# jfdev001/algebraic-multigrid

Hardware: AMD Instinct MI355X
Metric: V-cycles/sec, 2D Poisson N=4096^2 (fine-grid smoother HBM GB/s under roofline) (higher is better)
Workload: dtype f64; 1 GPU; 2D 5-point Poisson 4096x4096 (Grid::laplacian/rhs), true Jacobi smoother omega=0.6 2+2 sweeps, 16-level V-cycle, coarsest 511 dofs, fp64, 1xMI355X; smoother has no counterpart in the reference: pinned to the oracle twin; n=4096, dim=2, levels=16, smoother=jacobi, sweeps=2, graph=True, coarse_solve=band-chain (LDS-resident scalar recurrence, half-bandwidth <= 3, bit-exact), layout=dict

## Files before the change

algebraic-multigrid_amd/csrc/kernels.hip:

```cpp
#include <hip/hip_runtime.h>
#include <cstdlib>
#include <stdint.h>

#include <cstdio>
#include <type_traits>
#include <utility>
#include <vector>
#include <algorithm>
#include <cmath>

#include "kernels.hpp"

namespace amg_hip {

__device__ __forceinline__ void lds_barrier() {
  asm volatile("s_waitcnt lgkmcnt(0)\n\ts_barrier" ::: "memory");
}

constexpr bool mode_cheb(int m) { return (m & ~3) == 16; }
constexpr bool mode_jac(int m) { return m == CSR_JACOBI || mode_cheb(m); }
constexpr bool cheb_first(int m) { return (m & 1) != 0; }
constexpr bool cheb_last(int m) { return (m & 2) != 0; }
template <int MODE>
__device__ __forceinline__ double cheb_update(double t, double xi, double di, double alpha, double beta,
// ... 250 lines not shown
      else { if (v > w[2]) w[2] = v; }
    }
  }
#pragma unroll
  for (int a = 0; a < 3; ++a) red[a][threadIdx.x] = w[a];
  __syncthreads();
  for (int h = 128; h > 0; h >>= 1) {
    if ((int)threadIdx.x < h) {
#pragma unroll
      for (int a = 0; a < 3; ++a) red[a][threadIdx.x] = fmax(red[a][threadIdx.x], red[a][threadIdx.x + h]);
    }
    __syncthreads();
  }
  if (threadIdx.x < 3) atomicMax(out + threadIdx.x, (unsigned long long)__double_as_longlong(red[threadIdx.x][0]));
}
__global__ void axis_strength_init_kernel(unsigned long long* out) {
  if (threadIdx.x < 3) out[threadIdx.x] = 0ull;
}
hipError_t launch_axis_strength(int64_t n, int dim, const int64_t dims[3], const int32_t* rowptr, const int32_t* col,
                                const double* val, uint64_t* out, hipStream_t st) {
  if ((dim != 2 && dim != 3) || !dims || dims[0] < 1 || dims[1] < 1 || dims[2] < 1 ||
      n != dims[0] * dims[1] * dims[2] || n >= ((int64_t)1 << 31))
    return hipErrorInvalidValue;
  hipLaunchKernelGGL(axis_strength_init_kernel, dim3(1), dim3(64), 0, st, reinterpret_cast<unsigned long long*>(out));
  hipError_t e = hipGetLastError();
  if (e != hipSuccess) return e;
  hipLaunchKernelGGL(axis_strength_kernel, dim3((unsigned)((n + 255) / 256)), dim3(256), 0, st, (uint32_t)n,
                     (uint32_t)dims[0], (uint32_t)dims[1], rowptr, col, val, reinterpret_cast<unsigned long long*>(out));
  return hipGetLastError();
}

template <int MODE, bool IDX16, bool NT>
__global__ __launch_bounds__(256) void sell_kernel(
    int n, const int64_t* __restrict__ soff, const void* __restrict__ scol_v,
    const double* __restrict__ sval, const double* x, const double* __restrict__ f,
    double* out, double omega, const int32_t* __restrict__ rowid, int row0,
    const double* __restrict__ uH, int nH, int dshift, double* dvec, double alpha) {
  auto corrected = [&](int c) -> double {
    const double xc = x[c];
    const int j = c >> 1;
    const double a = uH[(j >= 1 && j - 1 < nH) ? j - 1 : 0];
    const double b = uH[j < nH ? j : 0];
    double t = 0.0;
    if (c & 1) {
      if (j < nH) t += 1.0 * b;
    } else {
      if (j >= 1 && j - 1 < nH) t += 0.5 * a;
      if (j < nH) t += 0.5 * b;
    }
    return xc + t;
  };
  const int32_t* __restrict__ scol = static_cast<const int32_t*>(scol_v);
  const int16_t* __restrict__ scol16 = static_cast<const int16_t*>(scol_v);
  const int p = row0 + blockIdx.x * 256 + threadIdx.x;
  const int s = p >> 6;
  if ((s << 6) >= n) return;
  const int64_t o0 = soff[s], o1 = soff[s + 1];
  const int w = (int)((o1 - o0) >> 6);
  const int64_t base = o0 + (p & 63);
  int row = p;
  bool live = p < n;
  if (MODE == CSR_GS) {
    row = live ? rowid[p] : -1;
    live = row >= 0;
  }
  const int drow = row + dshift;
  double fi = 0.0, xi = 0.0, di = 0.0;
  if (live) {
    if (MODE != CSR_SPMV) fi = NT ? __builtin_nontemporal_load(f + row) : f[row];
    if (mode_jac(MODE) || MODE == CSR_GS) xi = x[drow];
    if (MODE == CSR_JACOBI_P) xi = corrected(row);
    if (mode_cheb(MODE) && !cheb_first(MODE)) di = NT ? __builtin_nontemporal_load(dvec + row) : dvec[row];
  }
  double acc = (MODE == CSR_RESID) ? fi : 0.0;
  double diag = 0.0;
  auto pass = [&](int j0, auto UU) {
    constexpr int UN = decltype(UU)::value;
    int32_t c[UN];
    double v[UN], xx[UN];
#pragma unroll
    for (int u = 0; u < UN; ++u) {
      const int j = j0 + u < w ? j0 + u : j0;
      const int64_t at = base + ((int64_t)j << 6);
      if (IDX16) {
        const int d = NT ? __builtin_nontemporal_load(scol16 + at) : scol16[at];
        c[u] = (d == -32768) ? -1 : drow + d;
      } else {
        c[u] = NT ? __builtin_nontemporal_load(scol + at) : scol[at];
      }
      v[u] = NT ? __builtin_nontemporal_load(sval + at) : sval[at];
    }
#pragma unroll
    for (int u = 0; u < UN; ++u) {
      if (MODE == CSR_JACOBI_P) xx[u] = corrected(c[u] >= 0 ? c[u] : 0);
      else xx[u] = x[c[u] >= 0 ? c[u] : 0];
    }
#pragma unroll
    for (int u = 0; u < UN; ++u) {
      if (j0 + u < w && c[u] >= 0) {
        if (MODE == CSR_RESID) {
          acc -= v[u] * xx[u];
        } else if (mode_jac(MODE) || MODE == CSR_GS || MODE == CSR_JACOBI_P) {
          if (c[u] == drow) diag = v[u];
          else acc += v[u] * xx[u];
        } else {
          acc += v[u] * xx[u];
        }
      }
    }
  };
  if (w == 0) {
  } else if (w <= 3) pass(0, std::integral_constant<int, 3>{});
  else if (w <= 5) pass(0, std::integral_constant<int, 5>{});
  else if (w <= 7) pass(0, std::integral_constant<int, 7>{});
  else if (w <= 9) pass(0, std::integral_constant<int, 9>{});
  else
    for (int j0 = 0; j0 < w; j0 += 8) pass(j0, std::integral_constant<int, 8>{});
  if (live) {
    double res;
    bool store = true;
    if (MODE == CSR_RESID || MODE == CSR_SPMV) {
      res = acc;
    } else if (MODE == CSR_JACOBI || MODE == CSR_JACOBI_P) {
      res = (diag == 0.0) ? xi : xi + omega * ((fi - acc) / diag - xi);
    } else if (mode_cheb(MODE)) {
      double dn;
      res = cheb_update<MODE>((diag == 0.0) ? xi : (fi - acc) / diag, xi, di, alpha, omega, dn);
      if (!cheb_last(MODE)) {
        if (NT) __builtin_nontemporal_store(dn, dvec + row);
        else dvec[row] = dn;
      }
    } else if (MODE == CSR_GS) {
      res = (fi - acc) / diag;
      store = diag != 0.0;
    } else {
      const double d = fi - acc;
      res = d * d;
    }
    if (store) {
      if (NT && MODE != CSR_GS) __builtin_nontemporal_store(res, out + row);
      else out[row] = res;
    }
  }
}

template <int MODE>
static hipError_t launch_sell_mode(int64_t n, int idx16, const int64_t* soff,
                                   const void* scol, const double* sval, const double* x,
                                   const double* f, double* out, double omega,
                                   const int32_t* rowid, int64_t row0, int64_t count,
                                   const double* uH, int64_t nH, hipStream_t st,
                                   int64_t diag_shift = 0, double* dvec = nullptr, double alpha = 0.0) {
  const unsigned grid = (unsigned)((count + 255) / 256);
#define AMG_SELL_LAUNCH(I16, NTF)                                                              \
  hipLaunchKernelGGL((sell_kernel<MODE, I16, NTF>), dim3(grid), dim3(256), 0, st, (int)n, soff, \
                     scol, sval, x, f, out, omega, rowid, (int)row0, uH, (int)nH, (int)diag_shift, dvec, alpha)
  switch (idx16 & 3) {
    case 0: AMG_SELL_LAUNCH(false, false); break;
    case 1: AMG_SELL_LAUNCH(true, false); break;
    case 2: AMG_SELL_LAUNCH(false, true); break;
    default: AMG_SELL_LAUNCH(true, true); break;
  }
#undef AMG_SELL_LAUNCH
  return hipGetLastError();
}
hipError_t launch_sell(int mode, int64_t n, int idx16, const int64_t* soff,
                       const void* scol, const double* sval, const double* x,
                       const double* f, double* out, double omega, int64_t diag_shift,
                       hipStream_t st) {
  if (n <= 0) return hipSuccess;
  if (n >= ((int64_t)1 << 31) - 256 || diag_shift >= ((int64_t)1 << 30)) return hipErrorInvalidValue;
  switch (mode) {
    case CSR_RESID: return launch_sell_mode<CSR_RESID>(n, idx16, soff, scol, sval, x, f, out, omega, nullptr, 0, n, nullptr, 0, st, diag_shift);
    case CSR_JACOBI: return launch_sell_mode<CSR_JACOBI>(n, idx16, soff, scol, sval, x, f, out, omega, nullptr, 0, n, nullptr, 0, st, diag_shift);
    case CSR_SPMV: return launch_sell_mode<CSR_SPMV>(n, idx16, soff, scol, sval, x, f, out, omega, nullptr, 0, n, nullptr, 0, st, diag_shift);
    case CSR_RSSQ: return launch_sell_mode<CSR_RSSQ>(n, idx16, soff, scol, sval, x, f, out, omega, nullptr, 0, n, nullptr, 0, st, diag_shift);
  }
  return hipErrorInvalidValue;
}

hipError_t launch_sell_cheb(int64_t n, int idx16, const int64_t* soff, const void* scol, const double* sval,
                            const double* x, const double* f, double* out, const ChebStep& c, hipStream_t st) {
  if (n <= 0) return hipSuccess;
  if (n >= ((int64_t)1 << 31) - 256 || !c.d || x == out) return hipErrorInvalidValue;
#define AMG_SELL_CHEB(FI, LA)                                                                                \
  return launch_sell_mode<cheb_kernel_mode(FI, LA)>(n, idx16, soff, scol, sval, x, f, out, c.beta, nullptr, 0, n, \
                                                    nullptr, 0, st, 0, c.d, c.alpha)
  if (c.first && c.last) AMG_SELL_CHEB(true, true);
  if (c.first) AMG_SELL_CHEB(true, false);
  if (c.last) AMG_SELL_CHEB(false, true);
  AMG_SELL_CHEB(false, false);
#undef AMG_SELL_CHEB
}

hipError_t launch_sell_jacobi_prolong(int64_t n, int idx16, const int64_t* soff,
                                      const void* scol, const double* sval, const double* u,
                                      const double* uH, int64_t nH, const double* f, double* out,
                                      double omega, hipStream_t st) {
  if (n <= 0) return hipSuccess;
  if (n >= ((int64_t)1 << 31) - 256 || nH < 1) return hipErrorInvalidValue;
  return launch_sell_mode<CSR_JACOBI_P>(n, idx16, soff, scol, sval, u, f, out, omega, nullptr,
                                        0, n, uH, nH, st);
}

hipError_t launch_sell_gs_color(int64_t n_storage, int ,
                                const int64_t* soff, const int32_t* scol, const double* sval,
                                const int32_t* rowid,
                                int64_t row0, int64_t count, const double* f, double* u,
                                hipStream_t st) {
  if (count <= 0) return hipSuccess;
  if (n_storage >= ((int64_t)1 << 31) - 256 || (row0 & 63)) return hipErrorInvalidValue;
  const int64_t end = row0 + count < n_storage ? row0 + count : n_storage;
  return launch_sell_mode<CSR_GS>(end, 0, soff, scol, sval, u, f, u, 1.0, rowid, row0,
                                  count, nullptr, 0, st);
}

static int g_dict_rows_per_lane = 2;
static int g_xcd_map = 1;
template <int WORDS, int R>
struct DictStream {
  uint64_t cw[R][2];
  uint32_t ty;
  double fi[R], xi[R];
  double di[R];
  bool live[R];
};
template <int MODE, int WORDS, bool NT, int R>
__device__ __forceinline__ void dict_fetch(DictStream<WORDS, R>& s, int row0, int n,
                                           const uint64_t* __restrict__ codes,
                                           const uint8_t* __restrict__ rtype,
                                           const double* __restrict__ f, const double* x,
                                           int dshift, const double* __restrict__ dvec = nullptr) {
  typedef uint64_t u64x2 __attribute__((ext_vector_type(2)));
  typedef double f64x2 __attribute__((ext_vector_type(2)));
  constexpr bool read_d = mode_cheb(MODE) && !cheb_first(MODE);
#pragma unroll
  for (int r = 0; r < R; ++r) {
    s.live[r] = row0 + r < n;
    s.cw[r][0] = s.cw[r][1] = ~(uint64_t)0;
    s.fi[r] = s.xi[r] = s.di[r] = 0.0;
  }
  s.ty = 0xFFFFu;
  if (R == 2 && s.live[R - 1]) {
    if (rtype) {
      s.ty = *reinterpret_cast<const uint16_t*>(rtype + row0);
    } else {
      const u64x2* vp = reinterpret_cast<const u64x2*>(codes + (int64_t)row0 * WORDS);
      const u64x2 a = NT ? __builtin_nontemporal_load(vp) : *vp;
      if (WORDS == 2) {
        const u64x2 b2 = NT ? __builtin_nontemporal_load(vp + 1) : vp[1];
        s.cw[0][0] = a.x; s.cw[0][1] = a.y; s.cw[R - 1][0] = b2.x; s.cw[R - 1][1] = b2.y;
      } else {
        s.cw[0][0] = a.x; s.cw[R - 1][0] = a.y;
      }
    }
    if (MODE != CSR_SPMV) {
      const f64x2* fp = reinterpret_cast<const f64x2*>(f + row0);
      const f64x2 t = NT ? __builtin_nontemporal_load(fp) : *fp;
      s.fi[0] = t.x; s.fi[R - 1] = t.y;
    }
    if (mode_jac(MODE)) { s.xi[0] = x[row0 + dshift]; s.xi[R - 1] = x[row0 + 1 + dshift]; }
    if (read_d) {
      const f64x2* dp = reinterpret_cast<const f64x2*>(dvec + row0);
      const f64x2 t = NT ? __builtin_nontemporal_load(dp) : *dp;
      s.di[0] = t.x; s.di[R - 1] = t.y;
    }
  } else if (s.live[0]) {
    if (rtype) {
      s.ty = 0xFF00u | rtype[row0];
    } else {
      const uint64_t* cp = codes + (int64_t)row0 * WORDS;
      if (WORDS == 2) {
        const u64x2* vp = reinterpret_cast<const u64x2*>(cp);
        const u64x2 t = NT ? __builtin_nontemporal_load(vp) : *vp;
        s.cw[0][0] = t.x; s.cw[0][1] = t.y;
      } else {
        s.cw[0][0] = NT ? __builtin_nontemporal_load(cp) : cp[0];
      }
    }
    if (MODE != CSR_SPMV) s.fi[0] = NT ? __builtin_nontemporal_load(f + row0) : f[row0];
    if (mode_jac(MODE)) s.xi[0] = x[row0 + dshift];
    if (read_d) s.di[0] = NT ? __builtin_nontemporal_load(dvec + row0) : dvec[row0];
  }
}
template <int WORDS>
__device__ __forceinline__ void dict_stage_words(uint64_t* wtab, const uint64_t* __restrict__ rwords) {
#pragma unroll
  for (int k = 0; k < WORDS; ++k) wtab[threadIdx.x * WORDS + k] = rwords[threadIdx.x * WORDS + k];
}
template <int WORDS, int R>
__device__ __forceinline__ void dict_expand(DictStream<WORDS, R>& s, const uint64_t* wtab) {
#pragma unroll
  for (int r = 0; r < R; ++r)
#pragma unroll
    for (int k = 0; k < WORDS; ++k) s.cw[r][k] = wtab[((s.ty >> (8 * r)) & 0xFFu) * WORDS + k];
}
struct DictEntry {
  double a;
  double d;
  int32_t off8;
  int32_t pad[3];
};
template <int MODE>
__device__ __forceinline__ void dict_stage_table(DictEntry* tab, const int32_t* __restrict__ doff,
                                                 const double* __restrict__ dval, int ntab) {
  const int t = threadIdx.x;
  const double v = t < ntab ? dval[t] : 0.0;
  const int32_t o = t < ntab ? doff[t] : 0;
  DictEntry e;
  constexpr bool split = mode_jac(MODE) || MODE == CSR_GS;
  e.a = (split && o == 0) ? 0.0 : v;
  e.d = (split && o == 0 && t < ntab) ? v : 0.0;
  e.off8 = o * 8;
  e.pad[0] = e.pad[1] = e.pad[2] = 0;
  tab[t] = e;
}
template <int MODE, int WORDS, int UN, int R>
__device__ __forceinline__ void dict_rows(const DictStream<WORDS, R>& s, int row0,
                                          const DictEntry* tab, const double* x, double omega,
                                          int dshift, double (&res)[R]) {
  uint32_t c8[R][UN];
  double v[R][UN], vd[R][UN], xx[R][UN];
  bool ok[R][UN];
  const char* xb = reinterpret_cast<const char*>(x);
#pragma unroll
  for (int r = 0; r < R; ++r) {
    const uint32_t drow8 = s.live[r] ? (uint32_t)(row0 + r + dshift) * 8u : 0u;
    const uint32_t w32[4] = {(uint32_t)s.cw[r][0], (uint32_t)(s.cw[r][0] >> 32),
                             (uint32_t)s.cw[r][1], (uint32_t)(s.cw[r][1] >> 32)};
#pragma unroll
    for (int u = 0; u < UN; ++u) {
      const uint32_t code = (w32[u >> 2] >> (8 * (u & 3))) & 0xFFu;
      ok[r][u] = code != 0xFFu;
      c8[r][u] = drow8 + (uint32_t)tab[code].off8;
      v[r][u] = tab[code].a;
      vd[r][u] = (mode_jac(MODE) || MODE == CSR_GS) ? tab[code].d : 0.0;
    }
  }
#pragma unroll
  for (int r = 0; r < R; ++r)
#pragma unroll
    for (int u = 0; u < UN; ++u)
      xx[r][u] = *reinterpret_cast<const double*>(xb + c8[r][u]);
#pragma unroll
  for (int r = 0; r < R; ++r) {
    double acc = (MODE == CSR_RESID) ? s.fi[r] : 0.0;
    double diag = 0.0;
#pragma unroll
    for (int u = 0; u < UN; ++u) {
      double t = v[r][u] * xx[r][u];
      if (mode_jac(MODE) || MODE == CSR_GS) {
        acc += t;
        diag += vd[r][u];
      } else {
        asm volatile("" : "+v"(t));
        t = ok[r][u] ? t : 0.0;
        if (MODE == CSR_RESID) acc -= t;
        else acc += t;
      }
    }
    if (MODE == CSR_RESID || MODE == CSR_SPMV) {
      res[r] = acc;
    } else if (mode_jac(MODE) || MODE == CSR_GS) {
      const bool nod = diag == 0.0;
      double q = (s.fi[r] - acc) / (nod ? 1.0 : diag);
      asm volatile("" : "+v"(q));
      if (MODE == CSR_GS || mode_cheb(MODE)) res[r] = nod ? s.xi[r] : q;
      else res[r] = nod ? s.xi[r] : s.xi[r] + omega * (q - s.xi[r]);
    } else {
      const double d = s.fi[r] - acc;
      res[r] = d * d;
    }
  }
}
template <int UN>
__device__ __forceinline__ bool dict_stencil_can(uint32_t ty, const bool (&live)[2],
                                                 const int32_t* __restrict__ uti) {
  constexpr int PAT = UN == 7 ? 7 : 15;
  const uint32_t t0 = (uint32_t)__builtin_amdgcn_readfirstlane((int)(ty & 0xFFu));
  const bool ok = ty == (t0 | (t0 << 8)) && live[0] && live[1];
  if (t0 == 255u || __builtin_amdgcn_ballot_w64(!ok) != 0) return false;
  return uti[t0 * 18u + 17u] == PAT;
}
template <int MODE, int UN>
__device__ __forceinline__ void dict_rows_stencil(uint32_t ty, const double (&fi)[2],
                                                  const double (&xi)[2], int row0,
                                                  const double* __restrict__ utd,
                                                  const int32_t* __restrict__ uti, const double* x,
                                                  double omega, double (&res)[2]) {
  static_assert(mode_jac(MODE) || MODE == CSR_RESID, "fast path of the hot modes");
  static_assert(UN == 7 || UN == 16, "7-point rows / 15-point rows");
  typedef double f64x2 __attribute__((ext_vector_type(2)));
  constexpr int PAT = UN == 7 ? 7 : 15;
  const uint32_t t0 = (uint32_t)__builtin_amdgcn_readfirstlane((int)(ty & 0xFFu));
  const int32_t* ti = uti + t0 * 18u;
  const double* td = utd + t0 * 33u + (MODE == CSR_RESID ? 16u : 0u);
  const double* xr = x + row0;
  double xx[2][PAT];
  if (PAT == 7) {
    const int g[4] = {0, 1, 5, 6};
#pragma unroll
    for (int k = 0; k < 4; ++k) {
      const f64x2 v = *reinterpret_cast<const f64x2*>(xr + ti[g[k]]);
      xx[0][g[k]] = v.x;
      xx[1][g[k]] = v.y;
    }
    const f64x2 c = *reinterpret_cast<const f64x2*>(xr);
    const double lo = xr[-1], hi = xr[2];
    xx[0][2] = lo;  xx[0][3] = c.x; xx[0][4] = c.y;
    xx[1][2] = c.x; xx[1][3] = c.y; xx[1][4] = hi;
  } else {
#pragma unroll
    for (int k = 0; k < 5; ++k) {
      const double* xc = xr + ti[3 * k + 1];
      const f64x2 c = *reinterpret_cast<const f64x2*>(xc);
      const double lo = xc[-1], hi = xc[2];
      xx[0][3 * k] = lo;  xx[0][3 * k + 1] = c.x; xx[0][3 * k + 2] = c.y;
      xx[1][3 * k] = c.x; xx[1][3 * k + 1] = c.y; xx[1][3 * k + 2] = hi;
    }
  }
#pragma unroll
  for (int r = 0; r < 2; ++r) {
    double acc = (MODE == CSR_RESID) ? fi[r] : 0.0;
#pragma unroll
    for (int u = 0; u < PAT; ++u) {
      const double t = td[u] * xx[r][u];
      if (mode_jac(MODE)) acc += t;
      else acc -= t;
    }
    if (MODE == CSR_RESID) {
      res[r] = acc;
    } else {
      const double diag = td[32];
      const bool nod = diag == 0.0;
      const double q = (fi[r] - acc) / (nod ? 1.0 : diag);
      if (mode_cheb(MODE)) res[r] = nod ? xi[r] : q;
      else res[r] = nod ? xi[r] : xi[r] + omega * (q - xi[r]);
    }
  }
}
template <int WORDS, bool NT, int R>
__device__ __forceinline__ void dict_store(const DictStream<WORDS, R>& s, int row0,
                                           const double (&res)[R], double* out) {
  typedef double f64x2 __attribute__((ext_vector_type(2)));
  if (R == 2 && s.live[R - 1]) {
    f64x2 t;
    t.x = res[0]; t.y = res[R - 1];
    f64x2* op = reinterpret_cast<f64x2*>(out + row0);
    if (NT) __builtin_nontemporal_store(t, op);
    else *op = t;
  } else if (s.live[0]) {
    if (NT) __builtin_nontemporal_store(res[0], out + row0);
    else out[row0] = res[0];
  }
}

__device__ __forceinline__ int xcd_tile(unsigned b, unsigned nb, int on) {
  if (!on) return (int)b;
  if (on >= 16) {
    const unsigned tp = (unsigned)on, s = tp >> 3;
    if (b >= nb / tp * tp) return (int)b;
    const unsigned k = b & 7u, i = b >> 3, p = i / s;
    return (int)(p * tp + k * s + (i - p * s));
  }
  const unsigned k = b & 7u, i = b >> 3, q = nb >> 3, r = nb & 7u;
  return (int)(k * q + (k < r ? k : r) + i);
}
template <int MODE, int WORDS, int UN, bool NT, int R>
__global__ __launch_bounds__(256) void dict_kernel(
    int n, const uint64_t* __restrict__ codes, const uint8_t* __restrict__ rtype,
    const uint64_t* __restrict__ rwords, const int32_t* __restrict__ doff,
    const double* __restrict__ dval, int ntab, const double* x, const double* __restrict__ f,
    double* out, double omega, int dshift, int xcd_map, const double* __restrict__ utd,
    const int32_t* __restrict__ uti, double* dvec, double alpha) {
  __shared__ DictEntry tab[256];
  __shared__ uint64_t wtab[256 * WORDS];
  const int row0 = (xcd_tile(blockIdx.x, gridDim.x, xcd_map) * 256 + (int)threadIdx.x) * R;
  DictStream<WORDS, R> s;
  dict_fetch<MODE, WORDS, NT, R>(s, row0, n, codes, rtype, f, x, dshift, dvec);
  dict_stage_table<MODE>(tab, doff, dval, ntab);
  if (rtype) dict_stage_words<WORDS>(wtab, rwords);
  __syncthreads();
  double res[R];
  bool fast = false;
  if constexpr ((mode_jac(MODE) || MODE == CSR_RESID) && R == 2 && (UN == 7 || UN == 16)) {
    if (utd) fast = dict_stencil_can<UN>(s.ty, s.live, uti);
    if (fast) dict_rows_stencil<MODE, UN>(s.ty, s.fi, s.xi, row0, utd, uti, x, omega, res);
  }
  if (!fast) {
    if (rtype) dict_expand<WORDS, R>(s, wtab);
    dict_rows<MODE, WORDS, UN, R>(s, row0, tab, x, omega, dshift, res);
  }
  if constexpr (mode_cheb(MODE)) {
    double dn[R];
#pragma unroll
    for (int r = 0; r < R; ++r) res[r] = cheb_update<MODE>(res[r], s.xi[r], s.di[r], alpha, omega, dn[r]);
    if (!cheb_last(MODE)) dict_store<WORDS, NT, R>(s, row0, dn, dvec);
  }
  dict_store<WORDS, NT, R>(s, row0, res, out);
}

template <int R>
__device__ __forceinline__ void dict_restrict_tail(int tile, int n, const double* rs, int nH,
                                                   double* __restrict__ fH,
                                                   const double* __restrict__ diagH,
                                                   double* __restrict__ uH1,
                                                   double* __restrict__ uH0, double omega) {
  for (int q = threadIdx.x; q < 128 * R - 1; q += 256) {
    const int j = tile * (128 * R - 1) + q;
    if (j >= nH) break;
    const int64_t i = 2 * (int64_t)j;
    double sum = 0.0;
    if (i < n) sum += 0.5 * rs[2 * q];
    if (i + 1 < n) sum += 1.0 * rs[2 * q + 1];
    if (i + 2 < n) sum += 0.5 * rs[2 * q + 2];
    fH[j] = sum;
    if (uH1) {
      const double xi = 0.0, acc = 0.0;
      const double d = diagH[j];
      uH1[j] = (d == 0.0) ? xi : xi + omega * ((sum - acc) / d - xi);
    } else {
      uH0[j] = 0.0;
    }
  }
}
template <int R>
__device__ __forceinline__ void dict_prolong_tail(int tile, int n, const double* rs, int n_h,
                                                  const double* uh_in, double* uh_out) {
  typedef double f64x2 __attribute__((ext_vector_type(2)));
  const int stride = 256 * R - 2;
#pragma unroll
  for (int r = 0; r < R; ++r) {
    const int q = (int)threadIdx.x * R + r;
    const int j = tile * stride + q;
    if ((q == 0 && tile != 0) || q > stride || j > n) continue;
    double t0 = 0.0, t1 = 0.0;
    const double b = (j < n) ? rs[q] : 0.0;
    if (j >= 1 && j - 1 < n) t0 += 0.5 * rs[q - 1];
    if (j < n) {
      t0 += 0.5 * b;
      t1 += 1.0 * b;
    }
    const int64_t i = 2 * (int64_t)j;
    if (i + 1 < n_h) {
      f64x2 u = *reinterpret_cast<const f64x2*>(uh_in + i);
      u.x = u.x + t0;
      u.y = u.y + t1;
      *reinterpret_cast<f64x2*>(uh_out + i) = u;
    } else if (i < n_h) {
      uh_out[i] = uh_in[i] + t0;
    }
  }
}
template <int WORDS, int UN, bool NT, int R>
__global__ __launch_bounds__(256) void dict_resid_restrict_kernel(
    int n, const uint64_t* __restrict__ codes, const uint8_t* __restrict__ rtype,
    const uint64_t* __restrict__ rwords, const int32_t* __restrict__ doff,
    const double* __restrict__ dval, int ntab, const double* x, const double* __restrict__ f,
    double* r_out, int nH, double* __restrict__ fH, const double* __restrict__ diagH,
    double* __restrict__ uH1, double* __restrict__ uH0, double omega, int xcd_map,
    const double* __restrict__ utd, const int32_t* __restrict__ uti) {
  __shared__ DictEntry tab[256];
  __shared__ uint64_t wtab[256 * WORDS];
  __shared__ double rs[256 * R];
  const int tile = xcd_tile(blockIdx.x, gridDim.x, xcd_map);
  const int row0 = tile * (256 * R - 2) + (int)threadIdx.x * R;
  DictStream<WORDS, R> s;
  dict_fetch<CSR_RESID, WORDS, NT, R>(s, row0, n, codes, rtype, f, x, 0);
  dict_stage_table<CSR_RESID>(tab, doff, dval, ntab);
  if (rtype) dict_stage_words<WORDS>(wtab, rwords);
  __syncthreads();
  double res[R];
  bool fast = false;
  if constexpr (R == 2 && (UN == 7 || UN == 16)) {
    if (utd) fast = dict_stencil_can<UN>(s.ty, s.live, uti);
    if (fast) dict_rows_stencil<CSR_RESID, UN>(s.ty, s.fi, s.xi, row0, utd, uti, x, omega, res);
  }
  if (!fast) {
    if (rtype) dict_expand<WORDS, R>(s, wtab);
    dict_rows<CSR_RESID, WORDS, UN, R>(s, row0, tab, x, omega, 0, res);
  }
  if (r_out) dict_store<WORDS, NT, R>(s, row0, res, r_out);
#pragma unroll
  for (int r = 0; r < R; ++r) rs[threadIdx.x * R + r] = s.live[r] ? res[r] : 0.0;
  __syncthreads();
  dict_restrict_tail<R>(tile, n, rs, nH, fH, diagH, uH1, uH0, omega);
}
template <int WORDS, int UN, bool NT, int R>
__global__ __launch_bounds__(256) void dict_jacobi_prolong_kernel(
    int n, const uint64_t* __restrict__ codes, const uint8_t* __restrict__ rtype,
    const uint64_t* __restrict__ rwords, const int32_t* __restrict__ doff,
    const double* __restrict__ dval, int ntab, const double* x, const double* __restrict__ f,
    double* out, double omega, int n_h, const double* uh_in, double* uh_out, int xcd_map,
    const double* __restrict__ utd, const int32_t* __restrict__ uti) {
  __shared__ DictEntry tab[256];
  __shared__ uint64_t wtab[256 * WORDS];
  __shared__ double rs[256 * R];
  const int tile = xcd_tile(blockIdx.x, gridDim.x, xcd_map);
  const int stride = 256 * R - 2;
  const int row0 = tile * stride + (int)threadIdx.x * R;
  DictStream<WORDS, R> s;
  dict_fetch<CSR_JACOBI, WORDS, NT, R>(s, row0, n, codes, rtype, f, x, 0);
  dict_stage_table<CSR_JACOBI>(tab, doff, dval, ntab);
  if (rtype) dict_stage_words<WORDS>(wtab, rwords);
  __syncthreads();
  double res[R];
  bool fast = false;
  if constexpr (R == 2 && (UN == 7 || UN == 16)) {
    if (utd) fast = dict_stencil_can<UN>(s.ty, s.live, uti);
    if (fast) dict_rows_stencil<CSR_JACOBI, UN>(s.ty, s.fi, s.xi, row0, utd, uti, x, omega, res);
  }
  if (!fast) {
    if (rtype) dict_expand<WORDS, R>(s, wtab);
    dict_rows<CSR_JACOBI, WORDS, UN, R>(s, row0, tab, x, omega, 0, res);
  }
  dict_store<WORDS, NT, R>(s, row0, res, out);
#pragma unroll
  for (int r = 0; r < R; ++r) rs[threadIdx.x * R + r] = s.live[r] ? res[r] : 0.0;
  __syncthreads();
  dict_prolong_tail<R>(tile, n, rs, n_h, uh_in, uh_out);
}

constexpr int PAIR_HB = 66;
constexpr int PAIR_W = 512 + 2 * PAIR_HB;

template <int WORDS, int UN>
__device__ __forceinline__ void dict_pair_stage1(int n, int w0, int hbw, const uint64_t* codes,
                                                 const uint8_t* rtype, const DictEntry* tabJ,
                                                 const uint64_t* wtab, const double* a,
                                                 const double* f, double omega, double* uw,
                                                 double* u_out) {
  const int W = 512 + 2 * hbw;
  for (int base = 0; base < W; base += 512) {
    const int lw = base + (int)threadIdx.x * 2;
    const int row0 = w0 + lw;
    DictStream<WORDS, 2> s;
    const bool inside = row0 >= 0 && lw < W;
    dict_fetch<CSR_JACOBI, WORDS, false, 2>(s, inside ? row0 : 0, inside ? n : 0, codes, rtype, f, a, 0);
    if (rtype) dict_expand<WORDS, 2>(s, wtab);
    double res[2];
    dict_rows<CSR_JACOBI, WORDS, UN, 2>(s, row0, tabJ, a, omega, 0, res);
    if (lw < W) {
      uw[lw] = s.live[0] ? res[0] : 0.0;
      uw[lw + 1] = s.live[1] ? res[1] : 0.0;
    }
    if (u_out && lw >= hbw && lw < hbw + 512) dict_store<WORDS, false, 2>(s, row0, res, u_out);
  }
}
template <int WORDS, int UN>
__global__ __launch_bounds__(256) void dict_pair_down_kernel(
    int n, const uint64_t* __restrict__ codes, const uint8_t* __restrict__ rtype,
    const uint64_t* __restrict__ rwords, const int32_t* __restrict__ doff,
    const double* __restrict__ dval, int ntab, const double* a, const double* __restrict__ f,
    double* u_out, double* r_out, int nH, double* __restrict__ fH,
    const double* __restrict__ diagH, double* __restrict__ uH1, double omega, int hbw,
    int xcd_map) {
  __shared__ DictEntry tabJ[256];
  __shared__ DictEntry tabR[256];
  __shared__ uint64_t wtab[256 * WORDS];
  __shared__ double uw[PAIR_W];
  __shared__ double rs[512];
  const int tile = xcd_tile(blockIdx.x, gridDim.x, xcd_map);
  const int t0 = tile * 510, w0 = t0 - hbw;
  dict_stage_table<CSR_JACOBI>(tabJ, doff, dval, ntab);
  dict_stage_table<CSR_RESID>(tabR, doff, dval, ntab);
  if (rtype) dict_stage_words<WORDS>(wtab, rwords);
  __syncthreads();
  dict_pair_stage1<WORDS, UN>(n, w0, hbw, codes, rtype, tabJ, wtab, a, f, omega, uw, u_out);
  __syncthreads();
  const int row0 = t0 + (int)threadIdx.x * 2;
  DictStream<WORDS, 2> s;
  dict_fetch<CSR_RESID, WORDS, false, 2>(s, row0, n, codes, rtype, f, a, 0);
  if (rtype) dict_expand<WORDS, 2>(s, wtab);
  double res[2];
  dict_rows<CSR_RESID, WORDS, UN, 2>(s, row0 - w0, tabR, uw, omega, 0, res);
  if (r_out) dict_store<WORDS, false, 2>(s, row0, res, r_out);
  rs[threadIdx.x * 2] = s.live[0] ? res[0] : 0.0;
  rs[threadIdx.x * 2 + 1] = s.live[1] ? res[1] : 0.0;
  __syncthreads();
  dict_restrict_tail<2>(tile, n, rs, nH, fH, diagH, uH1, nullptr, omega);
}
template <int WORDS, int UN>
__global__ __launch_bounds__(256) void dict_pair_up_kernel(
    int n, const uint64_t* __restrict__ codes, const uint8_t* __restrict__ rtype,
    const uint64_t* __restrict__ rwords, const int32_t* __restrict__ doff,
    const double* __restrict__ dval, int ntab, const double* a, const double* __restrict__ f,
    double* u_out, double omega, int hbw, int n_h, const double* uh_in, double* uh_out,
    int xcd_map) {
  __shared__ DictEntry tabJ[256];
  __shared__ uint64_t wtab[256 * WORDS];
  __shared__ double uw[PAIR_W];
  __shared__ double rs[512];
  const int tile = xcd_tile(blockIdx.x, gridDim.x, xcd_map);
  const int t0 = tile * 510, w0 = t0 - hbw;
  dict_stage_table<CSR_JACOBI>(tabJ, doff, dval, ntab);
  if (rtype) dict_stage_words<WORDS>(wtab, rwords);
  __syncthreads();
  dict_pair_stage1<WORDS, UN>(n, w0, hbw, codes, rtype, tabJ, wtab, a, f, omega, uw, nullptr);
  __syncthreads();
  const int row0 = t0 + (int)threadIdx.x * 2;
  DictStream<WORDS, 2> s;
  dict_fetch<CSR_RESID, WORDS, false, 2>(s, row0, n, codes, rtype, f, a, 0);
  s.xi[0] = uw[row0 - w0];
  s.xi[1] = uw[row0 - w0 + 1];
  if (rtype) dict_expand<WORDS, 2>(s, wtab);
  double res[2];
  dict_rows<CSR_JACOBI, WORDS, UN, 2>(s, row0 - w0, tabJ, uw, omega, 0, res);
  dict_store<WORDS, false, 2>(s, row0, res, u_out);
  rs[threadIdx.x * 2] = s.live[0] ? res[0] : 0.0;
  rs[threadIdx.x * 2 + 1] = s.live[1] ? res[1] : 0.0;
  __syncthreads();
  dict_prolong_tail<2>(tile, n, rs, n_h, uh_in, uh_out);
}

constexpr int PATCH_TW = 64;
constexpr int PATCH_TH = 42;
constexpr int PATCH_EH = PATCH_TH + 6;
constexpr int PATCH_EC = PATCH_TW + 8;
constexpr int PATCH_NT = 432;
constexpr int PATCH_K = PATCH_EH * PATCH_EC / PATCH_NT;
constexpr int PATCH_BUF = (PATCH_EH + 2) * PATCH_EC;
constexpr int PATCH_MAXTAB = 192;
static_assert(PATCH_EH * PATCH_EC == PATCH_K * PATCH_NT && PATCH_NT % PATCH_EC == 0, "patch geometry");

struct PatchJ { double a, d; };
struct PatchR { double a; int32_t loff, ok; };

struct PatchCells {
  int cell0, row0, lj0, li;
  double f[PATCH_K];
  uint32_t ty[PATCH_K];
  bool live[PATCH_K];
  bool uniform;
  uint32_t tu;
};

struct PatchU {
  double wj[9], wr[9], diag;
#ifdef AMG_PATCH_FASTDIV
  double rdiag;
#endif
  uint32_t rmask, corners;
};
__device__ __forceinline__ void patch_load_u(PatchU& U, uint32_t tu, const double* __restrict__ utabd,
                                             const int32_t* __restrict__ utabi) {
  const double* d = utabd + (size_t)tu * 19;
  const int32_t* i = utabi + (size_t)tu * 2;
#pragma unroll
  for (int e = 0; e < 9; ++e) {
    U.wj[e] = d[e];
    U.wr[e] = d[9 + e];
  }
  U.diag = d[18];
#ifdef AMG_PATCH_FASTDIV
  U.rdiag = 1.0 / (U.diag == 0.0 ? 1.0 : U.diag);
#endif
  U.rmask = (uint32_t)i[0];
  U.corners = (uint32_t)i[1];
}
template <bool RESID, bool CORNERS, bool GS = false, int MASK = -1>
__device__ __forceinline__ void patch_eval_u(const double* buf, int cell0, const PatchU& U,
                                             const double (&f)[PATCH_K], double omega,
                                             double (&res)[PATCH_K]) {
  const double* p = buf + cell0 - PATCH_EC;
  if (!CORNERS && !RESID && U.diag == 0.0) {
#pragma unroll
    for (int k = 0; k < PATCH_K; ++k) res[k] = p[(k + 1) * PATCH_EC];
    return;
  }
  double w[3][3];
#pragma unroll
  for (int r = 0; r < 2; ++r)
#pragma unroll
    for (int c = 0; c < 3; ++c) w[r][c] = (CORNERS || c == 1 || r == 1) ? p[r * PATCH_EC + c - 1] : 0.0;
#pragma unroll
  for (int k = 0; k < PATCH_K; ++k) {
#pragma unroll
    for (int c = 0; c < 3; ++c)
      w[2][c] = (CORNERS || c == 1) ? p[(k + 2) * PATCH_EC + c - 1] : 0.0;
    if (!CORNERS) {
      w[2][0] = p[(k + 2) * PATCH_EC - 1];
      w[2][2] = p[(k + 2) * PATCH_EC + 1];
    }
    const double xi = w[1][1];
    if (RESID) {
      double acc = f[k];
#pragma unroll
      for (int s9 = 0; s9 < 9; ++s9) {
        const int r = s9 / 3, c = s9 % 3;
        if (!CORNERS && r != 1 && c != 1) continue;
        if (MASK >= 0) {
          if ((MASK >> s9) & 1) acc -= U.wr[s9] * w[r][c];
        } else {
          double t = U.wr[s9] * w[r][c];
          t = ((U.rmask >> s9) & 1u) ? t : 0.0;
          acc -= t;
        }
      }
      res[k] = acc;
    } else {
      double acc = 0.0;
#pragma unroll
      for (int s9 = 0; s9 < 9; ++s9) {
        const int r = s9 / 3, c = s9 % 3;
        if (s9 == 4 || (!CORNERS && r != 1 && c != 1)) continue;
        if (MASK >= 0 && !((MASK >> s9) & 1)) continue;
        acc += U.wj[s9] * w[r][c];
      }
      if (CORNERS && U.diag == 0.0) {
        res[k] = xi;
      } else {
#ifdef AMG_PATCH_FASTDIV
        const double nm = f[k] - acc;
        const double q0 = nm * U.rdiag;
        const double r0 = __builtin_fma(-U.diag, q0, nm);
        const double q1 = __builtin_fma(r0, U.rdiag, q0);
        const double r1 = __builtin_fma(-U.diag, q1, nm);
        const double q = __builtin_fma(r1, U.rdiag, q1);
#else
        const double q = (f[k] - acc) / U.diag;
#endif
        res[k] = GS ? q : xi + omega * (q - xi);
      }
    }
#pragma unroll
    for (int c = 0; c < 3; ++c) {
      w[0][c] = w[1][c];
      w[1][c] = w[2][c];
    }
  }
}
template <int UN, bool RESID, bool GS = false>
__device__ __forceinline__ double patch_eval(const double* buf, int cell, uint32_t type,
                                             const PatchJ* tabJ, const PatchR* tabR, double fi,
                                             double omega) {
  const int t0 = (int)type * UN;
  double xx[UN];
  if (RESID) {
    double av[UN];
    bool ok[UN];
#pragma unroll
    for (int e = 0; e < UN; ++e) {
      const PatchR r = tabR[t0 + e];
      av[e] = r.a;
      ok[e] = r.ok != 0;
      xx[e] = buf[cell + r.loff];
    }
    double acc = fi;
#pragma unroll
    for (int e = 0; e < UN; ++e) {
      double t = av[e] * xx[e];
      t = ok[e] ? t : 0.0;
      acc -= t;
    }
    return acc;
  }
  double aj[UN], dj[UN];
#pragma unroll
  for (int e = 0; e < UN; ++e) {
    const PatchJ j = tabJ[t0 + e];
    aj[e] = j.a; dj[e] = j.d;
    xx[e] = buf[cell + tabR[t0 + e].loff];
  }
  double acc = 0.0, diag = 0.0;
  const double xi = buf[cell];
#pragma unroll
  for (int e = 0; e < UN; ++e) {
    acc += aj[e] * xx[e];
    diag += dj[e];
  }
  const bool nod = diag == 0.0;
  const double q = (fi - acc) / (nod ? 1.0 : diag);
  return nod ? xi : (GS ? q : xi + omega * (q - xi));
}

template <int UN, int UM, bool RESID, bool NT, bool ZERO>
__device__ __forceinline__ void patch_stage(const PatchCells& pc, int m, int ntypes, double* buf,
                                            const PatchU& U, const PatchJ* tabJ, const PatchR* tabR,
                                            double omega, int l0, int l1, int c0, int c1, double* out) {
  const bool inc = pc.li >= c0 && pc.li < c1;
  double res[PATCH_K];
  bool did[PATCH_K], inr[PATCH_K];
#pragma unroll
  for (int k = 0; k < PATCH_K; ++k) {
    const int lj = pc.lj0 + k;
    inr[k] = inc && lj >= l0 && lj < l1;
    did[k] = inr[k] && pc.live[k];
  }
  if (pc.uniform && U.rmask == (uint32_t)UM) {
    patch_eval_u<RESID, (UM & 0x145) != 0, false, (UM & 0x145) ? -1 : UM>(buf, pc.cell0, U, pc.f, omega, res);
  } else {
#pragma unroll
    for (int k = 0; k < PATCH_K; ++k)
      res[k] = patch_eval<UN, RESID>(buf, pc.cell0 + k * PATCH_EC,
                                     did[k] ? pc.ty[k] : (uint32_t)ntypes, tabJ, tabR, pc.f[k], omega);
  }
  lds_barrier();
  const bool outc = out != nullptr && pc.li >= 0 && pc.li < PATCH_TW;
#pragma unroll
  for (int k = 0; k < PATCH_K; ++k) {
    if (did[k]) buf[pc.cell0 + k * PATCH_EC] = res[k];
    else if (ZERO && inr[k]) buf[pc.cell0 + k * PATCH_EC] = 0.0;
    const int lj = pc.lj0 + k;
    if (outc && did[k] && lj >= 0 && lj < PATCH_TH) {
      double* op = out + (pc.row0 + k * m);
      if (NT) __builtin_nontemporal_store(res[k], op);
      else *op = res[k];
    }
  }
}

template <bool NT>
__device__ __forceinline__ void patch_copy_out(const double* buf, double* __restrict__ out, int n, int m,
                                               int j0, int i0) {
  for (int q = threadIdx.x; q < PATCH_TH * PATCH_TW; q += PATCH_NT) {
    const int lj = q / PATCH_TW, li = q - lj * PATCH_TW;
    const int64_t row = (int64_t)(j0 + lj) * m + i0 + li;
    if (row < (int64_t)n) {
      const double v = buf[(lj + 4) * PATCH_EC + li + 4];
      if (NT) __builtin_nontemporal_store(v, out + row);
      else out[row] = v;
    }
  }
}

struct __attribute__((aligned(8))) PatchPair { double x, y; };
template <bool PROLONG, bool UNI, bool XF = false>
__device__ __forceinline__ void patch_load(PatchCells& pc, uint32_t tf, int n, int m, int j0, int i0,
                                           const double* __restrict__ x,
                                           const double* __restrict__ f,
                                           const uint8_t* __restrict__ rtype, int ntypes,
                                           const double* __restrict__ uH, int nH, double* buf) {
  const int g = (int)threadIdx.x / PATCH_EC, col = (int)threadIdx.x - g * PATCH_EC;
  const int le = g * PATCH_K;
  pc.lj0 = le - 3;
  pc.li = col - 4;
  pc.cell0 = (le + 1) * PATCH_EC + col;
  const int64_t r0 = (int64_t)(j0 + pc.lj0) * m + i0 + pc.li;
  pc.row0 = (int)(r0 < -((int64_t)1 << 30) ? -((int64_t)1 << 30) : r0);
  uint32_t mism = 0;
  double xv[PATCH_K];
#pragma unroll
  for (int k = 0; k < PATCH_K; ++k) {
    const int64_t r64 = r0 + (int64_t)k * m;
    pc.live[k] = UNI || (r64 >= 0 && r64 < (int64_t)n);
    const int row = pc.live[k] ? (int)r64 : 0;
    if (!XF) xv[k] = x[row];
    pc.f[k] = f[row];
    pc.ty[k] = UNI ? tf : (uint32_t)rtype[row];
  }
#pragma unroll
  for (int k = 0; k < PATCH_K; ++k) {
    const int row = pc.row0 + k * m;
    double x0 = (!XF && pc.live[k]) ? xv[k] : 0.0;
    if (PROLONG) {
      const int j = pc.live[k] ? (row >> 1) : 0;
      const bool odd = (row & 1) != 0;
      const bool a_ok = pc.live[k] && !odd && j >= 1 && j - 1 < nH;
      const bool b_ok = pc.live[k] && j < nH;
      const int jc = j < 1 ? 1 : (j > nH - 1 ? nH - 1 : j);
      const PatchPair pr = *reinterpret_cast<const PatchPair*>(uH + (jc - 1));
      const double a = (j == jc) ? pr.x : pr.y;
      const double b = (j == jc) ? pr.y : pr.x;
      double t = 0.0;
      t = a_ok ? t + 0.5 * a : t;
      t = b_ok ? t + (odd ? 1.0 : 0.5) * b : t;
      x0 = pc.live[k] ? x0 + t : x0;
    }
    if (!XF) buf[pc.cell0 + k * PATCH_EC] = x0;
    const uint32_t nty = (uint32_t)ntypes;
    pc.ty[k] = (pc.live[k] && pc.ty[k] < nty) ? pc.ty[k] : nty;
    pc.f[k] = pc.live[k] ? pc.f[k] : 0.0;
  }
  if (UNI) {
    pc.tu = tf;
    pc.uniform = true;
    return;
  }
  pc.tu = (uint32_t)__builtin_amdgcn_readfirstlane((int)pc.ty[0]);
#pragma unroll
  for (int k = 0; k < PATCH_K; ++k) mism |= pc.ty[k] ^ pc.tu;
  pc.uniform = __builtin_amdgcn_ballot_w64(mism != 0) == 0 && pc.tu < (uint32_t)ntypes;
}

__global__ __launch_bounds__(256) void patch_tile_flags_kernel(int n, int m, int px_count,
                                                               const uint8_t* __restrict__ rtype,
                                                               int ntypes, uint8_t* __restrict__ flag) {
  const int tile = blockIdx.x;
  const int py = tile / px_count, px = tile - py * px_count;
  const int64_t base = (int64_t)(py * PATCH_TH - 3) * m + px * PATCH_TW - 4;
  const int64_t first = base < 0 ? 0 : (base < n ? base : n - 1);
  const uint32_t t0 = rtype[first];
  int ok = base >= 0 && t0 < (uint32_t)ntypes;
  for (int q = threadIdx.x; q < PATCH_EH * PATCH_EC; q += 256) {
    const int le = q / PATCH_EC, c = q - le * PATCH_EC;
    const int64_t r = base + (int64_t)le * m + c;
    ok = ok && r >= 0 && r < (int64_t)n && rtype[r < 0 ? 0 : (r < n ? r : n - 1)] == t0;
  }
  ok = __syncthreads_and(ok);
  if (threadIdx.x == 0) flag[tile] = ok ? (uint8_t)t0 : (uint8_t)255;
}
hipError_t launch_patch_tile_flags(int64_t n, int64_t m, const uint8_t* rtype, int ntypes, uint8_t* flag,
                                   int64_t* n_tiles, hipStream_t st) {
  if (!patch_geometry_ok(n, m)) return hipErrorInvalidValue;
  const int64_t lines = (n + m - 1) / m;
  const int pxc = (int)(m / PATCH_TW);
  const int64_t tiles = (lines + PATCH_TH - 1) / PATCH_TH * pxc;
  if (n_tiles) *n_tiles = tiles;
  if (!flag) return hipSuccess;
  hipLaunchKernelGGL(patch_tile_flags_kernel, dim3((unsigned)tiles), dim3(256), 0, st, (int)n, (int)m, pxc,
                     rtype, ntypes, flag);
  return hipGetLastError();
}

__global__ __launch_bounds__(256) void patch_coarse_flags_kernel(int n, int m, int px_count, int nH,
// ... 4801 lines not shown
```

Baseline: 1386 V-cycles/s.

## Stage pair-kernel window inputs into LDS with all global loads issued upfront

The pair down/up kernels now issue every global load up front into registers: table entries, row-type words, the x window with halo, f, codes, and the diagH or coarse-u values for the tails. They then commit these to LDS once, so both Jacobi stages read x, f and codes from shared memory instead of fetching them twice from global memory. Prefetching the restrict and prolong tail operands hides their latency behind the smoother work. The cost is much higher LDS and register use per block, which may lower occupancy. These pair kernels may only run on small coarse levels.

Result: faster. 1412 V-cycles/s, median of 6 (+1.9%).

```diff
diff --git a/algebraic-multigrid_amd/csrc/kernels.hip b/algebraic-multigrid_amd/csrc/kernels.hip
--- a/algebraic-multigrid_amd/csrc/kernels.hip
+++ b/algebraic-multigrid_amd/csrc/kernels.hip
@@ -576,11 +576,8 @@
   int32_t pad[3];
 };
 template <int MODE>
-__device__ __forceinline__ void dict_stage_table(DictEntry* tab, const int32_t* __restrict__ doff,
-                                                 const double* __restrict__ dval, int ntab) {
+__device__ __forceinline__ void dict_put_table(DictEntry* tab, double v, int32_t o, int ntab) {
   const int t = threadIdx.x;
-  const double v = t < ntab ? dval[t] : 0.0;
-  const int32_t o = t < ntab ? doff[t] : 0;
   DictEntry e;
   constexpr bool split = mode_jac(MODE) || MODE == CSR_GS;
   e.a = (split && o == 0) ? 0.0 : v;
@@ -588,6 +585,14 @@
   e.off8 = o * 8;
   e.pad[0] = e.pad[1] = e.pad[2] = 0;
   tab[t] = e;
+}
+template <int MODE>
+__device__ __forceinline__ void dict_stage_table(DictEntry* tab, const int32_t* __restrict__ doff,
+                                                 const double* __restrict__ dval, int ntab) {
+  const int t = threadIdx.x;
+  const double v = t < ntab ? dval[t] : 0.0;
+  const int32_t o = t < ntab ? doff[t] : 0;
+  dict_put_table<MODE>(tab, v, o, ntab);
 }
 template <int MODE, int WORDS, int UN, int R>
 __device__ __forceinline__ void dict_rows(const DictStream<WORDS, R>& s, int row0,
@@ -823,6 +828,72 @@
       *reinterpret_cast<f64x2*>(uh_out + i) = u;
     } else if (i < n_h) {
       uh_out[i] = uh_in[i] + t0;
+    }
+  }
+}
+__device__ __forceinline__ double dict_restrict_pre(int tile, int nH, const double* __restrict__ diagH) {
+  const int q = threadIdx.x, j = tile * 255 + q;
+  return (q < 255 && j < nH) ? diagH[j] : 0.0;
+}
+__device__ __forceinline__ void dict_restrict_tail(int tile, int n, const double* rs, int nH,
+                                                   double* __restrict__ fH, double dH,
+                                                   double* __restrict__ uH1, double omega) {
+  const int q = threadIdx.x, j = tile * 255 + q;
+  if (q >= 255 || j >= nH) return;
+  const int64_t i = 2 * (int64_t)j;
+  double sum = 0.0;
+  if (i < n) sum += 0.5 * rs[2 * q];
+  if (i + 1 < n) sum += 1.0 * rs[2 * q + 1];
+  if (i + 2 < n) sum += 0.5 * rs[2 * q + 2];
+  fH[j] = sum;
+  const double xi = 0.0, acc = 0.0;
+  const double d = dH;
+  uH1[j] = (d == 0.0) ? xi : xi + omega * ((sum - acc) / d - xi);
+}
+typedef double pair_f64x2 __attribute__((ext_vector_type(2)));
+__device__ __forceinline__ void dict_prolong_pre(int tile, int n, int n_h, const double* uh_in,
+                                                 pair_f64x2 (&pre)[2], double& lone) {
+  bool two[2], one[2];
+  int64_t i[2];
+#pragma unroll
+  for (int r = 0; r < 2; ++r) {
+    const int q = (int)threadIdx.x * 2 + r;
+    const int j = tile * 510 + q;
+    const bool on = !((q == 0 && tile != 0) || q > 510 || j > n);
+    i[r] = 2 * (int64_t)j;
+    two[r] = on && i[r] + 1 < n_h;
+    one[r] = on && i[r] + 1 == n_h;
+    pre[r].x = pre[r].y = 0.0;
+  }
+  lone = 0.0;
+#pragma unroll
+  for (int r = 0; r < 2; ++r)
+    if (two[r]) pre[r] = *reinterpret_cast<const pair_f64x2*>(uh_in + i[r]);
+  if (one[0] || one[1]) lone = uh_in[n_h - 1];
+}
+__device__ __forceinline__ void dict_prolong_tail(int tile, int n, const double* rs, int n_h,
+                                                  const pair_f64x2 (&pre)[2], double lone,
+                                                  double* uh_out) {
+#pragma unroll
+  for (int r = 0; r < 2; ++r) {
+    const int q = (int)threadIdx.x * 2 + r;
+    const int j = tile * 510 + q;
+    if ((q == 0 && tile != 0) || q > 510 || j > n) continue;
+    double t0 = 0.0, t1 = 0.0;
+    const double b = (j < n) ? rs[q] : 0.0;
+    if (j >= 1 && j - 1 < n) t0 += 0.5 * rs[q - 1];
+    if (j < n) {
+      t0 += 0.5 * b;
+      t1 += 1.0 * b;
+    }
+    const int64_t i = 2 * (int64_t)j;
+    if (i + 1 < n_h) {
+      pair_f64x2 u = pre[r];
+      u.x = u.x + t0;
+      u.y = u.y + t1;
+      *reinterpret_cast<pair_f64x2*>(uh_out + i) = u;
+    } else if (i < n_h) {
+      uh_out[i] = lone + t0;
     }
   }
 }
@@ -897,23 +968,160 @@
 
 constexpr int PAIR_HB = 66;
 constexpr int PAIR_W = 512 + 2 * PAIR_HB;
+constexpr int PAIR_AW = PAIR_W + 2 * PAIR_HB;
+constexpr int PAIR_AP = (PAIR_AW / 2 + 255) / 256;
+static_assert(PAIR_W <= 1024 && PAIR_HB % 2 == 0, "two passes of 512 rows cover the window");
+
+typedef uint64_t pair_u64x2 __attribute__((ext_vector_type(2)));
+template <int WORDS>
+struct PairLoads {
+  double tv;
+  int32_t to;
+  uint64_t rw[WORDS];
+  pair_f64x2 a[PAIR_AP];
+  pair_f64x2 f[2];
+  double fl[2];
+  uint32_t ty[2], tl[2];
+  pair_u64x2 c[2][WORDS], cl[2];
+};
+template <int WORDS, bool TYPES>
+__device__ __forceinline__ void dict_pair_issue(PairLoads<WORDS>& g, int n, int w0, int hbw,
+                                                const uint64_t* __restrict__ codes,
+                                                const uint8_t* __restrict__ rtype,
+                                                const uint64_t* __restrict__ rwords,
+                                                const int32_t* __restrict__ doff,
+                                                const double* __restrict__ dval, int ntab,
+                                                const double* a, const double* __restrict__ f) {
+  const int t = threadIdx.x;
+  const int W = 512 + 2 * hbw, AW = W + 2 * hbw;
+  g.tv = t < ntab ? dval[t] : 0.0;
+  g.to = t < ntab ? doff[t] : 0;
+#pragma unroll
+  for (int k = 0; k < WORDS; ++k) g.rw[k] = TYPES ? rwords[t * WORDS + k] : 0;
+#pragma unroll
+  for (int k = 0; k < PAIR_AP; ++k) {
+    const int idx = (k * 256 + t) * 2;
+    const int row = w0 - hbw + idx;
+    g.a[k].x = g.a[k].y = 0.0;
+    if (idx < AW && row >= 0) {
+      if (row + 1 < n) g.a[k] = *reinterpret_cast<const pair_f64x2*>(a + row);
+      else if (row < n) g.a[k].x = a[row];
+    }
+  }
+  bool both[2], lone[2];
+#pragma unroll
+  for (int k = 0; k < 2; ++k) {
+    const int lw = (k * 256 + t) * 2, row0 = w0 + lw;
+    const bool inside = row0 >= 0 && lw < W;
+    both[k] = inside && row0 + 1 < n;
+    lone[k] = inside && row0 + 1 == n;
+    g.f[k].x = g.f[k].y = g.fl[k] = 0.0;
+    if (both[k]) g.f[k] = *reinterpret_cast<const pair_f64x2*>(f + row0);
+    if (lone[k]) g.fl[k] = f[row0];
+  }
+#pragma unroll
+  for (int k = 0; k < 2; ++k) {
+    const int row0 = w0 + (k * 256 + t) * 2;
+    if (TYPES) {
+      g.ty[k] = 0xFFFFu;
+      g.tl[k] = 0xFFu;
+      if (both[k]) g.ty[k] = *reinterpret_cast<const uint16_t*>(rtype + row0);
+      if (lone[k]) g.tl[k] = rtype[row0];
+    } else {
+      g.cl[k].x = g.cl[k].y = ~(uint64_t)0;
+#pragma unroll
+      for (int j = 0; j < WORDS; ++j) g.c[k][j].x = g.c[k][j].y = ~(uint64_t)0;
+      const uint64_t* cp = codes + (int64_t)row0 * WORDS;
+      if (both[k]) {
+#pragma unroll
+        for (int j = 0; j < WORDS; ++j) g.c[k][j] = reinterpret_cast<const pair_u64x2*>(cp)[j];
+      }
+      if (lone[k]) {
+        if (WORDS == 2) g.cl[k] = *reinterpret_cast<const pair_u64x2*>(cp);
+        else g.cl[k].x = cp[0];
+      }
+    }
+  }
+}
+template <int WORDS, bool TYPES>
+__device__ __forceinline__ void dict_pair_commit(const PairLoads<WORDS>& g, int n, int w0, int hbw,
+                                                 uint64_t* wc, uint16_t* tw, double* aw,
+                                                 double* fw) {
+  const int t = threadIdx.x;
+  const int W = 512 + 2 * hbw, AW = W + 2 * hbw;
+  if (TYPES) {
+#pragma unroll
+    for (int k = 0; k < WORDS; ++k) wc[t * WORDS + k] = g.rw[k];
+  }
+#pragma unroll
+  for (int k = 0; k < PAIR_AP; ++k) {
+    const int idx = (k * 256 + t) * 2;
+    if (idx < AW) *reinterpret_cast<pair_f64x2*>(aw + idx) = g.a[k];
+  }
+#pragma unroll
+  for (int k = 0; k < 2; ++k) {
+    const int lw = (k * 256 + t) * 2;
+    if (lw >= W) continue;
+    const bool both = w0 + lw >= 0 && w0 + lw + 1 < n;
+    pair_f64x2 fv = g.f[k];
+    fv.x = both ? fv.x : g.fl[k];
+    *reinterpret_cast<pair_f64x2*>(fw + lw) = fv;
+    if (TYPES) {
+      uint32_t tl = g.tl[k];
+      asm volatile("" : "+v"(tl));
+      tw[lw >> 1] = (uint16_t)(both ? g.ty[k] : (tl | 0xFF00u));
+    } else {
+      pair_u64x2* wp = reinterpret_cast<pair_u64x2*>(wc + lw * WORDS);
+      wp[0] = both ? g.c[k][0] : g.cl[k];
+      if (WORDS == 2) wp[1] = g.c[k][WORDS - 1];
+    }
+  }
+}
+template <int WORDS>
+__device__ __forceinline__ void dict_pair_stream(DictStream<WORDS, 2>& s, int lw, int W, int row0, int n,
+                                                 bool types, const uint64_t* wc, const uint16_t* tw,
+                                                 const double* fw) {
+  const bool inside = row0 >= 0 && lw < W;
+#pragma unroll
+  for (int r = 0; r < 2; ++r) {
+    s.live[r] = inside && row0 + r < n;
+    s.cw[r][0] = s.cw[r][1] = ~(uint64_t)0;
+    s.fi[r] = s.xi[r] = s.di[r] = 0.0;
+  }
+  s.ty = 0xFFFFu;
+  if (lw < W) {
+    const pair_f64x2 fv = *reinterpret_cast<const pair_f64x2*>(fw + lw);
+    s.fi[0] = fv.x; s.fi[1] = fv.y;
+    if (types) {
+      s.ty = tw[lw >> 1];
+    } else {
+#pragma unroll
+      for (int r = 0; r < 2; ++r)
+#pragma unroll
+        for (int j = 0; j < WORDS; ++j) s.cw[r][j] = wc[(lw + r) * WORDS + j];
+    }
+  }
+}
 
 template <int WORDS, int UN>
-__device__ __forceinline__ void dict_pair_stage1(int n, int w0, int hbw, const uint64_t* codes,
-                                                 const uint8_t* rtype, const DictEntry* tabJ,
-                                                 const uint64_t* wtab, const double* a,
-                                                 const double* f, double omega, double* uw,
+__device__ __forceinline__ void dict_pair_stage1(int n, int w0, int hbw, bool types,
+                                                 const DictEntry* tabJ, const uint64_t* wc,
+                                                 const uint16_t* tw, const double* aw,
+                                                 const double* fw, double omega, double* uw,
                                                  double* u_out) {
   const int W = 512 + 2 * hbw;
   for (int base = 0; base < W; base += 512) {
     const int lw = base + (int)threadIdx.x * 2;
     const int row0 = w0 + lw;
     DictStream<WORDS, 2> s;
-    const bool inside = row0 >= 0 && lw < W;
-    dict_fetch<CSR_JACOBI, WORDS, false, 2>(s, inside ? row0 : 0, inside ? n : 0, codes, rtype, f, a, 0);
-    if (rtype) dict_expand<WORDS, 2>(s, wtab);
+    dict_pair_stream<WORDS>(s, lw, W, row0, n, types, wc, tw, fw);
+    if (lw < W) {
+      s.xi[0] = aw[lw + hbw];
+      s.xi[1] = aw[lw + hbw + 1];
+    }
+    if (types) dict_expand<WORDS, 2>(s, wc);
     double res[2];
-    dict_rows<CSR_JACOBI, WORDS, UN, 2>(s, row0, tabJ, a, omega, 0, res);
+    dict_rows<CSR_JACOBI, WORDS, UN, 2>(s, lw + hbw, tabJ, aw, omega, 0, res);
     if (lw < W) {
       uw[lw] = s.live[0] ? res[0] : 0.0;
       uw[lw + 1] = s.live[1] ? res[1] : 0.0;
@@ -931,28 +1139,37 @@
     int xcd_map) {
   __shared__ DictEntry tabJ[256];
   __shared__ DictEntry tabR[256];
-  __shared__ uint64_t wtab[256 * WORDS];
+  __shared__ __attribute__((aligned(16))) uint64_t wc[PAIR_W * WORDS];
+  __shared__ uint16_t tw[PAIR_W / 2];
+  __shared__ __attribute__((aligned(16))) double aw[PAIR_AW];
+  __shared__ __attribute__((aligned(16))) double fw[PAIR_W];
   __shared__ double uw[PAIR_W];
   __shared__ double rs[512];
   const int tile = xcd_tile(blockIdx.x, gridDim.x, xcd_map);
-  const int t0 = tile * 510, w0 = t0 - hbw;
-  dict_stage_table<CSR_JACOBI>(tabJ, doff, dval, ntab);
-  dict_stage_table<CSR_RESID>(tabR, doff, dval, ntab);
-  if (rtype) dict_stage_words<WORDS>(wtab, rwords);
+  const int t0 = tile * 510, w0 = t0 - hbw, W = 512 + 2 * hbw;
+  const bool types = rtype != nullptr;
+  PairLoads<WORDS> g;
+  if (types) dict_pair_issue<WORDS, true>(g, n, w0, hbw, codes, rtype, rwords, doff, dval, ntab, a, f);
+  else dict_pair_issue<WORDS, false>(g, n, w0, hbw, codes, rtype, rwords, doff, dval, ntab, a, f);
+  const double dH = dict_restrict_pre(tile, nH, diagH);
+  dict_put_table<CSR_JACOBI>(tabJ, g.tv, g.to, ntab);
+  dict_put_table<CSR_RESID>(tabR, g.tv, g.to, ntab);
+  if (types) dict_pair_commit<WORDS, true>(g, n, w0, hbw, wc, tw, aw, fw);
+  else dict_pair_commit<WORDS, false>(g, n, w0, hbw, wc, tw, aw, fw);
   __syncthreads();
-  dict_pair_stage1<WORDS, UN>(n, w0, hbw, codes, rtype, tabJ, wtab, a, f, omega, uw, u_out);
+  dict_pair_stage1<WORDS, UN>(n, w0, hbw, types, tabJ, wc, tw, aw, fw, omega, uw, u_out);
   __syncthreads();
   const int row0 = t0 + (int)threadIdx.x * 2;
   DictStream<WORDS, 2> s;
-  dict_fetch<CSR_RESID, WORDS, false, 2>(s, row0, n, codes, rtype, f, a, 0);
-  if (rtype) dict_expand<WORDS, 2>(s, wtab);
+  dict_pair_stream<WORDS>(s, row0 - w0, W, row0, n, types, wc, tw, fw);
+  if (types) dict_expand<WORDS, 2>(s, wc);
   double res[2];
   dict_rows<CSR_RESID, WORDS, UN, 2>(s, row0 - w0, tabR, uw, omega, 0, res);
   if (r_out) dict_store<WORDS, false, 2>(s, row0, res, r_out);
   rs[threadIdx.x * 2] = s.live[0] ? res[0] : 0.0;
   rs[threadIdx.x * 2 + 1] = s.live[1] ? res[1] : 0.0;
   __syncthreads();
-  dict_restrict_tail<2>(tile, n, rs, nH, fH, diagH, uH1, nullptr, omega);
+  dict_restrict_tail(tile, n, rs, nH, fH, dH, uH1, omega);
 }
 template <int WORDS, int UN>
 __global__ __launch_bounds__(256) void dict_pair_up_kernel(
@@ -962,29 +1179,40 @@
     double* u_out, double omega, int hbw, int n_h, const double* uh_in, double* uh_out,
     int xcd_map) {
   __shared__ DictEntry tabJ[256];
-  __shared__ uint64_t wtab[256 * WORDS];
+  __shared__ __attribute__((aligned(16))) uint64_t wc[PAIR_W * WORDS];
+  __shared__ uint16_t tw[PAIR_W / 2];
+  __shared__ __attribute__((aligned(16))) double aw[PAIR_AW];
+  __shared__ __attribute__((aligned(16))) double fw[PAIR_W];
   __shared__ double uw[PAIR_W];
   __shared__ double rs[512];
   const int tile = xcd_tile(blockIdx.x, gridDim.x, xcd_map);
-  const int t0 = tile * 510, w0 = t0 - hbw;
-  dict_stage_table<CSR_JACOBI>(tabJ, doff, dval, ntab);
-  if (rtype) dict_stage_words<WORDS>(wtab, rwords);
+  const int t0 = tile * 510, w0 = t0 - hbw, W = 512 + 2 * hbw;
+  const bool types = rtype != nullptr;
+  PairLoads<WORDS> g;
+  if (types) dict_pair_issue<WORDS, true>(g, n, w0, hbw, codes, rtype, rwords, doff, dval, ntab, a, f);
+  else dict_pair_issue<WORDS, false>(g, n, w0, hbw, codes, rtype, rwords, doff, dval, ntab, a, f);
+  pair_f64x2 pre[2];
+  double pre1;
+  dict_prolong_pre(tile, n, n_h, uh_in, pre, pre1);
+  dict_put_table<CSR_JACOBI>(tabJ, g.tv, g.to, ntab);
+  if (types) dict_pair_commit<WORDS, true>(g, n, w0, hbw, wc, tw, aw, fw);
+  else dict_pair_commit<WORDS, false>(g, n, w0, hbw, wc, tw, aw, fw);
   __syncthreads();
-  dict_pair_stage1<WORDS, UN>(n, w0, hbw, codes, rtype, tabJ, wtab, a, f, omega, uw, nullptr);
+  dict_pair_stage1<WORDS, UN>(n, w0, hbw, types, tabJ, wc, tw, aw, fw, omega, uw, nullptr);
   __syncthreads();
   const int row0 = t0 + (int)threadIdx.x * 2;
   DictStream<WORDS, 2> s;
-  dict_fetch<CSR_RESID, WORDS, false, 2>(s, row0, n, codes, rtype, f, a, 0);
+  dict_pair_stream<WORDS>(s, row0 - w0, W, row0, n, types, wc, tw, fw);
   s.xi[0] = uw[row0 - w0];
   s.xi[1] = uw[row0 - w0 + 1];
-  if (rtype) dict_expand<WORDS, 2>(s, wtab);
+  if (types) dict_expand<WORDS, 2>(s, wc);
   double res[2];
   dict_rows<CSR_JACOBI, WORDS, UN, 2>(s, row0 - w0, tabJ, uw, omega, 0, res);
   dict_store<WORDS, false, 2>(s, row0, res, u_out);
   rs[threadIdx.x * 2] = s.live[0] ? res[0] : 0.0;
   rs[threadIdx.x * 2 + 1] = s.live[1] ? res[1] : 0.0;
   __syncthreads();
-  dict_prolong_tail<2>(tile, n, rs, n_h, uh_in, uh_out);
+  dict_prolong_tail(tile, n, rs, n_h, pre, pre1, uh_out);
 }
 
 constexpr int PATCH_TW = 64;
```
